# matiasrodlo/arxiv-rag

Hardware: AMD Instinct MI355X
Metric: chunks embedded/sec + QPS@top-10, all-mpnet-base-v2 768-d, 1/2/4/8 MI355X (higher is better)
Workload: dtype bf16

## Files before the change

arxiv_rag_amd/csrc/encoder_kernels.h:

```cpp
#pragma once
#include <type_traits>

#include "arx_common.h"

__global__ void scan_lens_kernel(const int32_t* __restrict__ lens, int32_t* __restrict__ cu, int n) {
    __shared__ int32_t part[1024];
    const int tid = threadIdx.x, nt = blockDim.x;
    const int per = (n + nt - 1) / nt;
    const int b0 = tid * per, b1 = min(n, b0 + per);
    int s = 0;
    for (int b = b0; b < b1; ++b) s += lens[b];
    part[tid] = s;
    __syncthreads();
    if (tid == 0) {
        int run = 0;
        for (int i = 0; i < nt; ++i) { int v = part[i]; part[i] = run; run += v; }
        cu[n] = run;
    }
    __syncthreads();
    int run = part[tid];
    for (int b = b0; b < b1; ++b) { cu[b] = run; run += lens[b]; }
}

template <int ARCH, bool SEG = false>
// ... 144 lines not shown
    constexpr int CPR = DH / 8;
    constexpr int RPB = 256 / (DH * 2);
    constexpr int KS = DH / 16;
    constexpr int DB = DH / 32;
    extern __shared__ __attribute__((aligned(16))) char smem[];

    const int b = blockIdx.z, h = blockIdx.y;
    const int t0 = cu[b];
    const int L = cu[b + 1] - t0;
    const int q0 = blockIdx.x * (32 * NW);
    if (q0 >= L) return;
    const int Lk = (L + 31) & ~31;
    const int tid = threadIdx.x, lane = tid & 63, wid = tid >> 6;
    const int64_t ld = 3 * (int64_t)H;
    const uint16_t* Qg = qkv + (int64_t)t0 * ld + h * DH;
    const uint16_t* Kg = Qg + H;
    const uint16_t* Vg = Qg + 2 * H;

    char* Ks = smem;
    uint16_t* Vt = reinterpret_cast<uint16_t*>(smem + AttnSmem<DH>::k_bytes(Lk));
    float* Bs = reinterpret_cast<float*>(smem + AttnSmem<DH>::k_bytes(Lk) + AttnSmem<DH>::vt_bytes(Lk));
    const int vts = AttnSmem<DH>::vt_stride(Lk);
    const int bst = AttnSmem<DH>::bias_stride(Lk);

    for (int cid = tid; cid < Lk * CPR; cid += NT) {
        const int row = cid / CPR, pc = cid % CPR;
        const int c = pc ^ ((row / RPB) & (CPR - 1));
        u32x4 kv = u32x4{0u, 0u, 0u, 0u}, vv = u32x4{0u, 0u, 0u, 0u};
        if (row < L) {
            kv = *reinterpret_cast<const u32x4*>(Kg + (int64_t)row * ld + c * 8);
            vv = *reinterpret_cast<const u32x4*>(Vg + (int64_t)row * ld + pc * 8);
        }
        *reinterpret_cast<u32x4*>(Ks + (int64_t)cid * 16) = kv;
        const int k16 = row & 15;
        const int pos = (row & ~15) + (((k16 >> 2) & 1) << 3) + ((k16 >> 3) << 2) + (k16 & 3);
#pragma unroll
        for (int e = 0; e < 4; ++e) {
            Vt[(pc * 8 + 2 * e) * vts + pos] = (uint16_t)(vv[e] & 0xffffu);
            Vt[(pc * 8 + 2 * e + 1) * vts + pos] = (uint16_t)(vv[e] >> 16);
        }
    }
    if (HAS_BIAS) {
        const float* bt = bias_tbl + (int64_t)h * ARX_BIAS_ROW + ARX_BIAS_CENTER;
        for (int i = tid; i < 4 * bst; i += NT) {
            const int c = i / bst, j = i % bst;
            int d = j + c - Lk;
            d = d < -ARX_BIAS_CENTER ? -ARX_BIAS_CENTER : (d > ARX_BIAS_CENTER ? ARX_BIAS_CENTER : d);
            Bs[i] = bt[d];
        }
    }
    __syncthreads();

    const int qw = q0 + wid * 32;
    if (qw >= L) return;
    const int ql = lane & 31, hh = lane >> 5;
    const int q = qw + ql;
    const int qc = q < L ? q : L - 1;
    bf16x8 qf[KS];
#pragma unroll
    for (int ks = 0; ks < KS; ++ks)
        qf[ks] = *reinterpret_cast<const bf16x8*>(Qg + (int64_t)qc * ld + ks * 16 + hh * 8);

    f32x16 o[DB];
#pragma unroll
    for (int d = 0; d < DB; ++d)
#pragma unroll
        for (int r = 0; r < 16; ++r) o[d][r] = 0.f;
    float m_run = -INFINITY, l_run = 0.f;

    const int bc = (4 - (qc & 3)) & 3;
    const float* brow = Bs + bc * bst + (Lk - qc - bc);
    const int krow_sw = ((ql / RPB) & (CPR - 1));

    const int nkt = Lk >> 5;
    for (int kt = 0; kt < nkt; ++kt) {
        f32x16 s;
#pragma unroll
        for (int r = 0; r < 16; ++r) s[r] = 0.f;
        const char* krow = Ks + (int64_t)(kt * 32 + ql) * (DH * 2);
#pragma unroll
        for (int ks = 0; ks < KS; ++ks) {
            const bf16x8 kf = *reinterpret_cast<const bf16x8*>(krow + (((2 * ks + hh) ^ krow_sw) << 4));
            s = __builtin_amdgcn_mfma_f32_32x32x16_bf16(kf, qf[ks], s, 0, 0, 0);
        }
        float mx = -INFINITY;
#pragma unroll
        for (int g4 = 0; g4 < 4; ++g4) {
            const int kb = kt * 32 + 8 * g4 + 4 * hh;
            f32x4 bv = f32x4{0.f, 0.f, 0.f, 0.f};
            if (HAS_BIAS) bv = *reinterpret_cast<const f32x4*>(brow + kb);
#pragma unroll
            for (int e = 0; e < 4; ++e) {
                float v = s[g4 * 4 + e] * scale_log2e + bv[e];
                v = (kb + e < L) ? v : -INFINITY;
                s[g4 * 4 + e] = v;
                mx = fmaxf(mx, v);
            }
        }
        mx = fmaxf(mx, __shfl_xor(mx, 32));
        const float m_new = fmaxf(m_run, mx);
        const float alpha = exp2f(m_run - m_new);
        m_run = m_new;
        float rs = 0.f;
#pragma unroll
        for (int r = 0; r < 16; ++r) { s[r] = exp2f(s[r] - m_new); rs += s[r]; }
        l_run = l_run * alpha + rs;
#pragma unroll
        for (int d = 0; d < DB; ++d)
#pragma unroll
            for (int r = 0; r < 16; ++r) o[d][r] *= alpha;
        bf16x8 pf[2];
#pragma unroll
        for (int ss = 0; ss < 2; ++ss)
#pragma unroll
            for (int e = 0; e < 8; ++e) pf[ss][e] = (bf16_t)s[8 * ss + e];
#pragma unroll
        for (int d = 0; d < DB; ++d) {
            const uint16_t* vrow = Vt + (int64_t)(d * 32 + ql) * vts + kt * 32 + hh * 8;
#pragma unroll
            for (int ss = 0; ss < 2; ++ss) {
                const bf16x8 vf = *reinterpret_cast<const bf16x8*>(vrow + ss * 16);
                o[d] = __builtin_amdgcn_mfma_f32_32x32x16_bf16(vf, pf[ss], o[d], 0, 0, 0);
            }
        }
    }
    const float l_tot = l_run + __shfl_xor(l_run, 32);
    const float inv = 1.0f / l_tot;
    if (q < L) {
        uint16_t* orow = ctx + (int64_t)(t0 + q) * H + h * DH;
#pragma unroll
        for (int d = 0; d < DB; ++d)
#pragma unroll
            for (int g4 = 0; g4 < 4; ++g4) {
                u32x2 w2;
                w2[0] = pack_bf16x2(o[d][g4 * 4 + 0] * inv, o[d][g4 * 4 + 1] * inv);
                w2[1] = pack_bf16x2(o[d][g4 * 4 + 2] * inv, o[d][g4 * 4 + 3] * inv);
                *reinterpret_cast<u32x2*>(orow + d * 32 + 8 * g4 + 4 * hh) = w2;
            }
    }
}

typedef short s16x4 __attribute__((ext_vector_type(4)));
template <int DH> struct AttnSmem2 {
    static __host__ __device__ int kv_bytes(int Lk) { return Lk * DH * 2; }
    static __host__ __device__ int bias_stride(int Lk) { return 2 * Lk + 8; }
    static __host__ __device__ int total(int Lk, bool has) { return 2 * kv_bytes(Lk) + (has ? 4 * (2 * Lk + 8) * 4 : 0); }
};

template <int DH> struct AttnSmem3 {
    static __host__ __device__ int kv_bytes(int Lk) { return Lk * DH * 2; }
    static __host__ __device__ int bias_stride(int Lk) { return ((2 * Lk + 8 + 63) & ~63) + 64; }
    static __host__ __device__ int total(int Lk, bool has) { return 2 * kv_bytes(Lk) + (has ? 4 * bias_stride(Lk) * 4 : 0); }
};
__device__ __forceinline__ int attn_bias_off(int c) { return c == 0 ? 0 : (c == 1 ? 20 : (c == 2 ? 36 : 52)); }

template <int DH, bool HAS_BIAS, int NW>
__global__ __launch_bounds__(NW * 64, NW / 2) void attention_tr_kernel(const uint16_t* __restrict__ qkv, uint16_t* __restrict__ ctx,
                                                                        const int32_t* __restrict__ cu,
                                                                        const float* __restrict__ bias_tbl, int H,
                                                                        float scale_log2e, int dev_word, unsigned long long* dev_stamps) {
    constexpr int NT = NW * 64;
    constexpr int CPR = DH / 8;
    constexpr int RPB = 256 / (DH * 2);
#ifdef ARX_DEV_VARIANTS
    const unsigned lin = blockIdx.x + gridDim.x * (blockIdx.y + gridDim.y * blockIdx.z);
    if (dev_stamps && threadIdx.x == 0) {
        dev_stamps[4 * lin] = wall_clock64();
        dev_stamps[4 * lin + 3] = ((unsigned long long)__builtin_amdgcn_s_getreg((31 << 11) | 20) << 32) | (unsigned)__builtin_amdgcn_s_getreg((31 << 11) | 4);
    }
#endif
    constexpr int KS = DH / 16;
    constexpr int DB = DH / 32;
    constexpr int ROWB = DH * 2;
    constexpr int RPI = NT / CPR;
    extern __shared__ __attribute__((aligned(16))) char smem[];
    const int b = blockIdx.z, h = blockIdx.y;
    const int t0 = cu[b];
    const int L = cu[b + 1] - t0;
    const int q0 = blockIdx.x * (32 * NW);
    if (q0 >= L) return;
    const int Lk = (L + 31) & ~31;
    const int tid = threadIdx.x, lane = tid & 63, wid = tid >> 6;
    const uint32_t ld = 3u * (uint32_t)H;
    const uint16_t* Qg = qkv + (int64_t)t0 * ld + h * DH;
    const uint16_t* Kg = Qg + H;
    const uint16_t* Vg = Qg + 2 * H;
    char* Ks = smem;
    char* Vs = smem + AttnSmem3<DH>::kv_bytes(Lk);
    float* Bs = reinterpret_cast<float*>(smem + 2 * AttnSmem3<DH>::kv_bytes(Lk));
    const int bst = AttnSmem3<DH>::bias_stride(Lk);

    const int ql = lane & 31, hh = lane >> 5;
    const int qw = q0 + wid * 32;
    const int q = qw + ql;
    const int qc = q < L ? q : L - 1;
    bf16x8 qf[KS];
#pragma unroll
    for (int ks = 0; ks < KS; ++ks)
        qf[ks] = *reinterpret_cast<const bf16x8*>(Qg + (uint32_t)qc * ld + ks * 16 + hh * 8);
    {
        static_assert(RPI % 16 == 0, "staging pass must keep the swizzle terms constant per thread");
        typedef __attribute__((address_space(3))) void lds_v;
        typedef const __attribute__((address_space(1))) void gbl_v;
        const int pc = tid % CPR, r0 = tid / CPR;
        const int kc = pc ^ ((r0 / RPB) & (CPR - 1));
        const int vc = (DH == 64) ? (pc ^ (((r0 >> 1) & 1) << 2)) : pc;
        uint32_t lo = (uint32_t)(tid & ~63) * 16;
        int LkS = Lk;
#ifdef ARX_DEV_VARIANTS
        if (dev_word == 5) LkS = 0;
#endif
        for (int row = r0; row < LkS; row += RPI, lo += NT * 16) {
            const uint32_t gr = (uint32_t)(row < L ? row : L - 1) * ld;
            __builtin_amdgcn_global_load_lds((gbl_v*)(Kg + gr + kc * 8), (lds_v*)(Ks + lo), 16, 0, 0);
            __builtin_amdgcn_global_load_lds((gbl_v*)(Vg + gr + vc * 8), (lds_v*)(Vs + lo), 16, 0, 0);
        }
    }
    if (HAS_BIAS) {
        const float* bt = bias_tbl + (int64_t)h * ARX_BIAS_ROW + ARX_BIAS_CENTER;
        const int span = 2 * Lk + 8;
        for (int i = tid; i < 4 * span; i += NT) {
            const int c = (i >= span) + (i >= 2 * span) + (i >= 3 * span), j = i - c * span;
            int d = j + c - Lk;
            d = d < -ARX_BIAS_CENTER ? -ARX_BIAS_CENTER : (d > ARX_BIAS_CENTER ? ARX_BIAS_CENTER : d);
            Bs[c * bst + attn_bias_off(c) + j] = bt[d];
        }
    }
    __syncthreads();
#ifdef ARX_DEV_VARIANTS
    if (dev_stamps && threadIdx.x == 0) dev_stamps[4 * lin + 1] = wall_clock64();
    if (dev_word == 3) {
        if (q < L && qf[0][0] == 0x7fc1 && qf[1 % KS][1] == 0x7fc2) ctx[(int64_t)(t0 + q) * H + h * DH] = 1;
        return;
    }
#endif

    if (qw >= L) return;
    f32x16 o[DB];
    auto lds_bases = [&](const float*& bb, const char* (&kb)[KS], const char* (&vb)[DB]) {
        int lane = threadIdx.x & 63;
        asm volatile("" : "+v"(lane));
        const int ql = lane & 31, hh = lane >> 5;
        int qc = q0 + wid * 32 + ql;
        qc = qc < L ? qc : L - 1;
        const int bc = (4 - (qc & 3)) & 3;
        bb = Bs + bc * bst + attn_bias_off(bc) + (Lk - qc - bc) + 4 * hh;
        const int krow_sw = ((ql / RPB) & (CPR - 1));
#pragma unroll
        for (int ks = 0; ks < KS; ++ks) kb[ks] = Ks + ql * ROWB + (((2 * ks + hh) ^ krow_sw) << 4);
        const int g16 = lane >> 4, q_ = (lane & 15) >> 2, p_ = lane & 3;
        const int vsw = (DH == 64) ? (((q_ >> 1) & 1) << 2) : 0;
#pragma unroll
        for (int d = 0; d < DB; ++d) {
            const int col = 32 * d + 16 * (g16 & 1) + 4 * p_;
            vb[d] = Vs + (4 * hh + q_) * ROWB + (((col >> 3) ^ vsw) << 4) + ((p_ & 1) << 3);
        }
    };
    typedef __attribute__((address_space(3))) s16x4 lds_s16x4;
    typedef short s16x8 __attribute__((ext_vector_type(8)));
    f32x4 lsum;
    const s16x4 one4 = s16x4{0x3f80, 0x3f80, 0x3f80, 0x3f80};
    const int nkt = Lk >> 5;
    const int nfull = (L & 31) ? nkt - 1 : nkt;
    float l_tot;

    bool redo = false;
#ifdef ARX_DEV_VARIANTS
    redo = dev_word == 6;
#endif
    if (!redo) {
#pragma unroll
        for (int d = 0; d < DB; ++d)
#pragma unroll
            for (int r = 0; r < 16; ++r) o[d][r] = 0.f;
        lsum = f32x4{0.f, 0.f, 0.f, 0.f};
        typedef const __attribute__((address_space(3))) char* lds_cptr;
        typedef const __attribute__((address_space(3))) float* lds_fptr;
        lds_fptr bp;
        lds_cptr kp[KS], vp[DB];
        {
            const float* bb;
            const char* kb[KS];
            const char* vb[DB];
            lds_bases(bb, kb, vb);
            bp = (lds_fptr)bb;
#pragma unroll
            for (int ks = 0; ks < KS; ++ks) kp[ks] = (lds_cptr)kb[ks];
#pragma unroll
            for (int d = 0; d < DB; ++d) vp[d] = (lds_cptr)vb[d];
        }
        bf16x8 kf[KS];
#pragma unroll
        for (int ks = 0; ks < KS; ++ks) kf[ks] = *reinterpret_cast<const __attribute__((address_space(3))) bf16x8*>(kp[ks]);
        auto advance = [&](int n) {
            bp += 32 * n;
            asm volatile("" : "+v"(bp));
#pragma unroll
            for (int ks = 0; ks < KS; ++ks) { kp[ks] += 32 * ROWB * n; asm volatile("" : "+v"(kp[ks])); }
#pragma unroll
            for (int d = 0; d < DB; ++d) { vp[d] += 32 * ROWB * n; asm volatile("" : "+v"(vp[d])); }
            __builtin_amdgcn_sched_barrier(0);
        };
        auto fast = [&](auto masked_tag, auto off_tag, int kt) {
            constexpr bool MASKED = decltype(masked_tag)::value;
            constexpr int OFF = decltype(off_tag)::value;
            f32x16 s;
#pragma unroll
            for (int r = 0; r < 16; ++r) s[r] = 0.f;
#pragma unroll
            for (int ks = 0; ks < KS; ++ks) s = __builtin_amdgcn_mfma_f32_32x32x16_bf16(kf[ks], qf[ks], s, 0, 0, 0);
            __builtin_amdgcn_sched_barrier(0);
            f32x4 bv[4];
#pragma unroll
            for (int g4 = 0; g4 < 4; ++g4) bv[g4] = HAS_BIAS ? *reinterpret_cast<const __attribute__((address_space(3))) f32x4*>(bp + OFF * 32 + 8 * g4) : f32x4{0.f, 0.f, 0.f, 0.f};
            s16x4 vt[DB][4];
#pragma unroll
            for (int d = 0; d < DB; ++d)
#pragma unroll
                for (int j = 0; j < 4; ++j) vt[d][j] = __builtin_amdgcn_ds_read_tr16_b64_v4i16((lds_s16x4*)(vp[d] + (OFF * 32 + 8 * j) * ROWB));
            __builtin_amdgcn_sched_barrier(0);
            typedef float f32x2 __attribute__((ext_vector_type(2)));
            const f32x2 sc2 = f32x2{scale_log2e, scale_log2e};
#pragma unroll
            for (int g4 = 0; g4 < 4; ++g4)
#pragma unroll
                for (int e = 0; e < 4; e += 2) {
                    f32x2 v = __builtin_elementwise_fma(f32x2{s[g4 * 4 + e], s[g4 * 4 + e + 1]}, sc2, f32x2{bv[g4][e], bv[g4][e + 1]});
                    if (MASKED) {
                        v[0] = (kt * 32 + 8 * g4 + 4 * hh + e < L) ? v[0] : -INFINITY;
                        v[1] = (kt * 32 + 8 * g4 + 4 * hh + e + 1 < L) ? v[1] : -INFINITY;
                    }
                    s[g4 * 4 + e] = v[0]; s[g4 * 4 + e + 1] = v[1];
                }
            __builtin_amdgcn_sched_barrier(0);
#pragma unroll
            for (int r = 0; r < 16; ++r) s[r] = __builtin_amdgcn_exp2f(s[r]);
            uint32_t pw[8];
#pragma unroll
            for (int j = 0; j < 8; ++j) pw[j] = pack_bf16x2(s[2 * j], s[2 * j + 1]);
            __builtin_amdgcn_sched_barrier(0);
            if (!MASKED) {
#pragma unroll
                for (int ks = 0; ks < KS; ++ks) kf[ks] = *reinterpret_cast<const __attribute__((address_space(3))) bf16x8*>(kp[ks] + (OFF + 1) * 32 * ROWB);
            }
            __builtin_amdgcn_sched_barrier(0);
            bf16x8 pf[2];
#pragma unroll
            for (int ss = 0; ss < 2; ++ss) pf[ss] = __builtin_bit_cast(bf16x8, u32x4{pw[4 * ss], pw[4 * ss + 1], pw[4 * ss + 2], pw[4 * ss + 3]});
#pragma unroll
            for (int j = 0; j < 4; ++j)
                lsum = __builtin_amdgcn_mfma_f32_4x4x4bf16_1k(one4, __builtin_bit_cast(s16x4, u32x2{pw[2 * j], pw[2 * j + 1]}), lsum, 0, 0, 0);
#pragma unroll
            for (int d = 0; d < DB; ++d)
#pragma unroll
                for (int ss = 0; ss < 2; ++ss) {
                    s16x8 v8;
#pragma unroll
                    for (int e = 0; e < 4; ++e) { v8[e] = vt[d][2 * ss][e]; v8[4 + e] = vt[d][2 * ss + 1][e]; }
                    o[d] = __builtin_amdgcn_mfma_f32_32x32x16_bf16(__builtin_bit_cast(bf16x8, v8), pf[ss], o[d], 0, 0, 0);
                }
            __builtin_amdgcn_sched_barrier(0);
        };
        int kt = 0;
        for (; kt + 2 <= nfull; kt += 2) {
            fast(std::false_type{}, std::integral_constant<int, 0>{}, kt);
            fast(std::false_type{}, std::integral_constant<int, 1>{}, kt + 1);
            advance(2);
        }
        if (kt < nfull) { fast(std::false_type{}, std::integral_constant<int, 0>{}, kt); advance(1); }
        if (nfull < nkt) fast(std::true_type{}, std::integral_constant<int, 0>{}, nkt - 1);
        l_tot = lsum[0] + __shfl_xor(lsum[0], 32);
        redo = !__all(l_tot > 0x1p-100f && l_tot < 0x1p100f);
    }
    if (redo) {
#pragma unroll
    for (int d = 0; d < DB; ++d)
#pragma unroll
        for (int r = 0; r < 16; ++r) o[d][r] = 0.f;
    float m_run = -INFINITY;
    const float* bptr;
    const char* kptr[KS];
    const char* vptr[DB];
    lds_bases(bptr, kptr, vptr);
    constexpr float THR = 8.0f;
    const float inv_scale = 1.0f / scale_log2e;
    lsum = f32x4{0.f, 0.f, 0.f, 0.f};
    auto tile = [&](auto masked_tag, auto first_tag, int kt) {
        constexpr bool MASKED = decltype(masked_tag)::value;
        constexpr bool FIRST = decltype(first_tag)::value;
        f32x16 s;
        const float s0 = FIRST ? 0.f : -m_run * inv_scale;
#pragma unroll
        for (int r = 0; r < 16; ++r) s[r] = s0;
#pragma unroll
        for (int ks = 0; ks < KS; ++ks) {
            const bf16x8 kf = *reinterpret_cast<const bf16x8*>(kptr[ks]);
            s = __builtin_amdgcn_mfma_f32_32x32x16_bf16(kf, qf[ks], s, 0, 0, 0);
        }
#pragma unroll
        for (int g4 = 0; g4 < 4; ++g4) {
            f32x4 bv = f32x4{0.f, 0.f, 0.f, 0.f};
            if (HAS_BIAS) bv = *reinterpret_cast<const f32x4*>(bptr + 8 * g4);
#pragma unroll
            for (int e = 0; e < 4; ++e) {
                float v = fmaf(s[g4 * 4 + e], scale_log2e, bv[e]);
                if (MASKED) v = (kt * 32 + 8 * g4 + 4 * hh + e < L) ? v : -INFINITY;
                s[g4 * 4 + e] = v;
            }
        }
        float mx = -INFINITY;
#pragma unroll
        for (int r = 0; r < 16; r += 2) mx = fmaxf(mx, fmaxf(s[r], s[r + 1]));
        mx = fmaxf(mx, __shfl_xor(mx, 32));
        if (FIRST) {
            m_run = mx;
#pragma unroll
            for (int r = 0; r < 16; ++r) s[r] -= mx;
        } else if (__any(mx > THR)) {
            const float d = fmaxf(mx, 0.f);
            const float alpha = __builtin_amdgcn_exp2f(-d);
            m_run += d;
#pragma unroll
            for (int r = 0; r < 16; ++r) s[r] -= d;
#pragma unroll
            for (int r = 0; r < 4; ++r) lsum[r] *= alpha;
#pragma unroll
            for (int dd = 0; dd < DB; ++dd)
#pragma unroll
                for (int r = 0; r < 16; ++r) o[dd][r] *= alpha;
        }
#pragma unroll
        for (int r = 0; r < 16; ++r) s[r] = __builtin_amdgcn_exp2f(s[r]);
        uint32_t pw[8];
#pragma unroll
        for (int j = 0; j < 8; ++j) pw[j] = pack_bf16x2(s[2 * j], s[2 * j + 1]);
        bf16x8 pf[2];
#pragma unroll
        for (int ss = 0; ss < 2; ++ss) pf[ss] = __builtin_bit_cast(bf16x8, u32x4{pw[4 * ss], pw[4 * ss + 1], pw[4 * ss + 2], pw[4 * ss + 3]});
#pragma unroll
        for (int j = 0; j < 4; ++j)
            lsum = __builtin_amdgcn_mfma_f32_4x4x4bf16_1k(one4, __builtin_bit_cast(s16x4, u32x2{pw[2 * j], pw[2 * j + 1]}), lsum, 0, 0, 0);
#pragma unroll
        for (int d = 0; d < DB; ++d) {
#pragma unroll
            for (int ss = 0; ss < 2; ++ss) {
                const s16x4 lo = __builtin_amdgcn_ds_read_tr16_b64_v4i16((lds_s16x4*)(vptr[d] + (16 * ss) * ROWB));
                const s16x4 hi = __builtin_amdgcn_ds_read_tr16_b64_v4i16((lds_s16x4*)(vptr[d] + (16 * ss + 8) * ROWB));
                s16x8 v8;
#pragma unroll
                for (int e = 0; e < 4; ++e) { v8[e] = lo[e]; v8[4 + e] = hi[e]; }
                o[d] = __builtin_amdgcn_mfma_f32_32x32x16_bf16(__builtin_bit_cast(bf16x8, v8), pf[ss], o[d], 0, 0, 0);
            }
        }
        bptr += 32;
#pragma unroll
        for (int ks = 0; ks < KS; ++ks) kptr[ks] += 32 * ROWB;
#pragma unroll
        for (int d = 0; d < DB; ++d) vptr[d] += 32 * ROWB;
    };
    if (nfull > 0) tile(std::false_type{}, std::true_type{}, 0); else tile(std::true_type{}, std::true_type{}, 0);
    for (int kt = 1; kt < nfull; ++kt) tile(std::false_type{}, std::false_type{}, kt);
    if (nfull < nkt && nkt > 1) tile(std::true_type{}, std::false_type{}, nkt - 1);
    l_tot = lsum[0] + __shfl_xor(lsum[0], 32);
    }

    const float inv = 1.0f / l_tot;
    u32x4 pc[DB][2];
#pragma unroll
    for (int d = 0; d < DB; ++d) {
        uint32_t w[4][2];
#pragma unroll
        for (int g4 = 0; g4 < 4; ++g4) {
            w[g4][0] = pack_bf16x2(o[d][g4 * 4 + 0] * inv, o[d][g4 * 4 + 1] * inv);
            w[g4][1] = pack_bf16x2(o[d][g4 * 4 + 2] * inv, o[d][g4 * 4 + 3] * inv);
        }
#pragma unroll
        for (int g = 0; g < 2; ++g)
#pragma unroll
            for (int k = 0; k < 2; ++k) {
                const auto sw = __builtin_amdgcn_permlane32_swap(w[g][k], w[g + 2][k], false, false);
                pc[d][g][k] = sw[0]; pc[d][g][2 + k] = sw[1];
            }
    }
    if (q < L) {
        uint16_t* orow = ctx + (int64_t)(t0 + q) * H + h * DH + 16 * hh;
#pragma unroll
        for (int d = 0; d < DB; ++d) {
            *reinterpret_cast<u32x4*>(orow + d * 32) = pc[d][0];
            *reinterpret_cast<u32x4*>(orow + d * 32 + 8) = pc[d][1];
        }
    }
#ifdef ARX_DEV_VARIANTS
    if (dev_stamps && (threadIdx.x & 63) == 0) atomicMax(&dev_stamps[4 * lin + 2], (unsigned long long)wall_clock64());
#endif
}

#ifdef ARX_DEV_VARIANTS
template <int DH, int NSLOT_ = 8> struct AttnRing {
    static constexpr int NT = 512, NSLOT = NSLOT_, AHEAD = NSLOT - 1, SLOT_KEYS = 64;
    static constexpr int ROWB = DH * 2;
    static constexpr int SLOT_BYTES = 2 * SLOT_KEYS * ROWB;
    static constexpr int GPS = SLOT_BYTES / (NT * 16);
    static_assert(GPS >= 1 && GPS * NT * 16 == SLOT_BYTES, "slot must be whole passes of the block");
    static __host__ __device__ int bias_stride(int C0) { return (2 * C0 + 8 + 52 + 63) & ~63; }
    static __host__ __device__ int total(int C0, bool has) { return NSLOT * SLOT_BYTES + (has ? 4 * bias_stride(C0) * 4 : 0); }
};

#define ARX_VMCNT_CASE(N) case N: asm volatile("s_waitcnt vmcnt(" #N ")" ::: "memory"); break;
#define ARX_VMCNT_CASE4(A, B, C_, D) ARX_VMCNT_CASE(A) ARX_VMCNT_CASE(B) ARX_VMCNT_CASE(C_) ARX_VMCNT_CASE(D)
__device__ __forceinline__ void attn_wait_vm(int n) {
    switch (n) {
    ARX_VMCNT_CASE4(0, 1, 2, 3) ARX_VMCNT_CASE4(4, 5, 6, 7) ARX_VMCNT_CASE4(8, 9, 10, 11) ARX_VMCNT_CASE4(12, 13, 14, 15)
    ARX_VMCNT_CASE4(16, 17, 18, 19) ARX_VMCNT_CASE4(20, 21, 22, 23) ARX_VMCNT_CASE4(24, 25, 26, 27) ARX_VMCNT_CASE4(28, 29, 30, 31)
    ARX_VMCNT_CASE4(32, 33, 34, 35) ARX_VMCNT_CASE4(36, 37, 38, 39) ARX_VMCNT_CASE4(40, 41, 42, 43) ARX_VMCNT_CASE(44)
    default: asm volatile("s_waitcnt vmcnt(0)" ::: "memory"); break;
    }
}
#undef ARX_VMCNT_CASE4
#undef ARX_VMCNT_CASE

template <int DH, int NSLOT> struct AttnStream {
    using R = AttnRing<DH, NSLOT>;
    static constexpr int NT = R::NT, ROWB = R::ROWB, SLOT_BYTES = R::SLOT_BYTES, GPS = R::GPS, CPR = DH / 8, RPB = 256 / R::ROWB;
    const uint16_t* qkv; const int32_t* cu; char* ring;
    int H, h, G, n_seqs;
    uint32_t ld;
    int p_b, p_t0, p_L, p_step, p_nqp, p_nsteps, p_slot, c_slot;
    int inflight, pend_st;
    unsigned st_bits;

    __device__ __forceinline__ void p_load_item() {
        p_L = 0; p_step = 0;
        while (p_b < n_seqs) {
            const __attribute__((address_space(4))) int32_t* cuc = (const __attribute__((address_space(4))) int32_t*)cu;
            const int t0 = cuc[p_b], L = cuc[p_b + 1] - t0;
            if (L > 0) { p_t0 = t0; p_L = L; p_nqp = L > 128 ? 2 : 1; p_nsteps = p_nqp + ((L + 63) >> 6); break; }
            p_b += G;
        }
    }
    __device__ __forceinline__ void issue_next() {
        const uint16_t* base = qkv + (int64_t)p_t0 * ld + h * DH;
        const bool isq = p_step < p_nqp;
        const int r0 = isq ? 128 * p_step : 64 * (p_step - p_nqp);
        int t = threadIdx.x;
        asm volatile("" : "+v"(t));
        char* dst = ring + p_slot * SLOT_BYTES + (__builtin_amdgcn_readfirstlane(t) & ~63) * 16;
#pragma unroll
        for (int it = 0; it < GPS; ++it) {
            const int cid = it * NT + t, r128 = cid / CPR, pcn = cid % CPR;
            int row, col0, c;
            if (isq) { row = r0 + r128; col0 = 0; c = pcn ^ ((r128 / RPB) & (CPR - 1)); }
            else if (r128 < 64) { row = r0 + r128; col0 = H; c = pcn ^ ((r128 / RPB) & (CPR - 1)); }
            else { row = r0 + r128 - 64; col0 = 2 * H; c = (DH == 64) ? (pcn ^ (((r128 >> 1) & 1) << 2)) : pcn; }
            row = row < p_L ? row : p_L - 1;
            __builtin_amdgcn_global_load_lds((const __attribute__((address_space(1))) void*)(base + (uint32_t)row * ld + col0 + c * 8),
                                             (__attribute__((address_space(3))) void*)(dst + it * NT * 16), 16, 0, 0);
        }
        if (pend_st) st_bits |= 1u << inflight;
        pend_st = 0;
        ++inflight;
        p_slot = (p_slot + 1) & (R::NSLOT - 1);
        if (++p_step == p_nsteps) { p_b += G; p_load_item(); }
    }
    __device__ __forceinline__ const char* step_begin() {
        attn_wait_vm((inflight - 1) * GPS + (DH / 8) * __builtin_popcount(st_bits >> 1) + pend_st);
        asm volatile("" ::: "memory");
        __builtin_amdgcn_s_barrier();
        asm volatile("" ::: "memory");
        st_bits >>= 1;
        --inflight;
        if (p_L > 0) issue_next();
        const char* slot = ring + c_slot * SLOT_BYTES;
        c_slot = (c_slot + 1) & (R::NSLOT - 1);
        return slot;
    }
};

template <int DH, bool HAS_BIAS, bool MASKED, bool first>
__device__ __forceinline__ void attn_ring_tile(const char* kbase, int k0, int v0, const bf16x8 (&qf)[DH / 16], f32x16 (&o)[DH / 32],
                                               f32x4& lsum, float& m_run, const float* bp, int kt, int hh, int L,
                                               float scale_log2e, float inv_scale) {
    constexpr int KS = DH / 16, DB = DH / 32, ROWB = DH * 2;
    constexpr float THR = 8.0f;
    typedef __attribute__((address_space(3))) s16x4 lds_s16x4;
    typedef short s16x8 __attribute__((ext_vector_type(8)));
    f32x16 s;
    const float s0 = first ? 0.f : -m_run * inv_scale;
#pragma unroll
    for (int r = 0; r < 16; ++r) s[r] = s0;
#pragma unroll
    for (int ks = 0; ks < KS; ++ks) {
        const bf16x8 kf = *reinterpret_cast<const bf16x8*>(kbase + (k0 ^ (ks << 5)));
        s = __builtin_amdgcn_mfma_f32_32x32x16_bf16(kf, qf[ks], s, 0, 0, 0);
    }
#pragma unroll
    for (int g4 = 0; g4 < 4; ++g4) {
        f32x4 bv = f32x4{0.f, 0.f, 0.f, 0.f};
        if (HAS_BIAS) bv = *reinterpret_cast<const f32x4*>(bp + 8 * g4);
#pragma unroll
        for (int e = 0; e < 4; ++e) {
            float v = fmaf(s[g4 * 4 + e], scale_log2e, bv[e]);
            if (MASKED) v = (kt * 32 + 8 * g4 + 4 * hh + e < L) ? v : -INFINITY;
            s[g4 * 4 + e] = v;
        }
    }
    float mx = -INFINITY;
#pragma unroll
    for (int r = 0; r < 16; r += 2) mx = fmaxf(mx, fmaxf(s[r], s[r + 1]));
    mx = fmaxf(mx, __shfl_xor(mx, 32));
    if (first) {
        m_run = mx;
#pragma unroll
        for (int r = 0; r < 16; ++r) s[r] -= mx;
    } else if (__any(mx > THR)) {
        const float d = fmaxf(mx, 0.f);
        const float alpha = __builtin_amdgcn_exp2f(-d);
        m_run += d;
#pragma unroll
        for (int r = 0; r < 16; ++r) s[r] -= d;
#pragma unroll
        for (int r = 0; r < 4; ++r) lsum[r] *= alpha;
#pragma unroll
        for (int dd = 0; dd < DB; ++dd)
#pragma unroll
            for (int r = 0; r < 16; ++r) o[dd][r] *= alpha;
    }
#pragma unroll
    for (int r = 0; r < 16; ++r) s[r] = __builtin_amdgcn_exp2f(s[r]);
    uint32_t pw[8];
#pragma unroll
    for (int j = 0; j < 8; ++j) pw[j] = pack_bf16x2(s[2 * j], s[2 * j + 1]);
    bf16x8 pf[2];
#pragma unroll
    for (int ss = 0; ss < 2; ++ss) pf[ss] = __builtin_bit_cast(bf16x8, u32x4{pw[4 * ss], pw[4 * ss + 1], pw[4 * ss + 2], pw[4 * ss + 3]});
    const s16x4 one4 = s16x4{0x3f80, 0x3f80, 0x3f80, 0x3f80};
#pragma unroll
    for (int j = 0; j < 4; ++j)
        lsum = __builtin_amdgcn_mfma_f32_4x4x4bf16_1k(one4, __builtin_bit_cast(s16x4, u32x2{pw[2 * j], pw[2 * j + 1]}), lsum, 0, 0, 0);
    const uint32_t vaddr = (uint32_t)(size_t)(const __attribute__((address_space(3))) char*)kbase + (uint32_t)v0;
#pragma unroll
    for (int d = 0; d < DB; ++d) {
        const uint32_t va = vaddr ^ (uint32_t)(d << 6);
        s16x4 vt[2][2];
#pragma unroll
        for (int ss = 0; ss < 2; ++ss) {
            asm volatile("ds_read_b64_tr_b16 %0, %1 offset:%2" : "=v"(vt[ss][0]) : "v"(va), "n"((16 * ss) * ROWB));
            asm volatile("ds_read_b64_tr_b16 %0, %1 offset:%2" : "=v"(vt[ss][1]) : "v"(va), "n"((16 * ss + 8) * ROWB));
        }
        asm volatile("s_waitcnt lgkmcnt(0)" : "+v"(vt[0][0]), "+v"(vt[0][1]), "+v"(vt[1][0]), "+v"(vt[1][1]) :: "memory");
#pragma unroll
        for (int ss = 0; ss < 2; ++ss) {
            s16x8 v8;
#pragma unroll
            for (int e = 0; e < 4; ++e) { v8[e] = vt[ss][0][e]; v8[4 + e] = vt[ss][1][e]; }
            o[d] = __builtin_amdgcn_mfma_f32_32x32x16_bf16(__builtin_bit_cast(bf16x8, v8), pf[ss], o[d], 0, 0, 0);
        }
    }
}

template <int DH, bool HAS_BIAS, int NSLOT>
__global__ __launch_bounds__(512, 2) void attention_ring_kernel(const uint16_t* __restrict__ qkv, uint16_t* __restrict__ ctx,
                                                                 const int32_t* __restrict__ cu,
                                                                 const float* __restrict__ bias_tbl, int H, int n_seqs,
                                                                 int C0, float scale_log2e) {
    using R = AttnRing<DH, NSLOT>;
    constexpr int NT = R::NT, ROWB = R::ROWB, SLOT_BYTES = R::SLOT_BYTES, GPS = R::GPS;
    constexpr int CPR = DH / 8;
    constexpr int RPB = 256 / ROWB;
    constexpr int KS = DH / 16;
    constexpr int DB = DH / 32;
    constexpr int NSTORE = DB * 4;
    static_assert((R::AHEAD - 1) * GPS + 4 * NSTORE <= 44, "attn_wait_vm covers AHEAD - 1 younger slot-loads plus four items' stores");
// ... 576 lines not shown
```

Measured before the change: 22410.

## Split attention K/V staging so first QK tile overlaps the V load

The attention prologue now issues all K loads before all V loads and fetches Q and bias values into registers with inline asm. It then waits only on the K portion (vmcnt of the V count) before the first barrier, so the first tile's QK^T, softmax and packing run while V is still in flight. A second barrier waits for V before the PV step, and the main loop is restructured into phase-tagged halves. The gain is overlap of global-to-LDS staging with compute, at the cost of an extra block barrier, hand-managed waitcnts, and assumptions about sequence length bounds (NB sized for 544 keys).

```diff
diff --git a/arxiv_rag_amd/csrc/encoder_kernels.h b/arxiv_rag_amd/csrc/encoder_kernels.h
--- a/arxiv_rag_amd/csrc/encoder_kernels.h
+++ b/arxiv_rag_amd/csrc/encoder_kernels.h
@@ -320,7 +320,20 @@
     static __host__ __device__ int bias_stride(int Lk) { return ((2 * Lk + 8 + 63) & ~63) + 64; }
     static __host__ __device__ int total(int Lk, bool has) { return 2 * kv_bytes(Lk) + (has ? 4 * bias_stride(Lk) * 4 : 0); }
 };
-__device__ __forceinline__ int attn_bias_off(int c) { return c == 0 ? 0 : (c == 1 ? 20 : (c == 2 ? 36 : 52)); }
+__device__ __forceinline__ int attn_bias_off(int c) { return c == 0 ? 0 : 16 * c + 4; }
+
+#define ARX_VMCNT_CASE(N) case N: asm volatile("s_waitcnt vmcnt(" #N ")" ::: "memory"); break;
+#define ARX_VMCNT_CASE4(A, B, C_, D) ARX_VMCNT_CASE(A) ARX_VMCNT_CASE(B) ARX_VMCNT_CASE(C_) ARX_VMCNT_CASE(D)
+__device__ __forceinline__ void attn_wait_vm(int n) {
+    switch (n) {
+    ARX_VMCNT_CASE4(0, 1, 2, 3) ARX_VMCNT_CASE4(4, 5, 6, 7) ARX_VMCNT_CASE4(8, 9, 10, 11) ARX_VMCNT_CASE4(12, 13, 14, 15)
+    ARX_VMCNT_CASE4(16, 17, 18, 19) ARX_VMCNT_CASE4(20, 21, 22, 23) ARX_VMCNT_CASE4(24, 25, 26, 27) ARX_VMCNT_CASE4(28, 29, 30, 31)
+    ARX_VMCNT_CASE4(32, 33, 34, 35) ARX_VMCNT_CASE4(36, 37, 38, 39) ARX_VMCNT_CASE4(40, 41, 42, 43) ARX_VMCNT_CASE(44)
+    default: asm volatile("s_waitcnt vmcnt(0)" ::: "memory"); break;
+    }
+}
+#undef ARX_VMCNT_CASE4
+#undef ARX_VMCNT_CASE
 
 template <int DH, bool HAS_BIAS, int NW>
 __global__ __launch_bounds__(NW * 64, NW / 2) void attention_tr_kernel(const uint16_t* __restrict__ qkv, uint16_t* __restrict__ ctx,
@@ -333,14 +346,15 @@
 #ifdef ARX_DEV_VARIANTS
     const unsigned lin = blockIdx.x + gridDim.x * (blockIdx.y + gridDim.y * blockIdx.z);
     if (dev_stamps && threadIdx.x == 0) {
-        dev_stamps[4 * lin] = wall_clock64();
-        dev_stamps[4 * lin + 3] = ((unsigned long long)__builtin_amdgcn_s_getreg((31 << 11) | 20) << 32) | (unsigned)__builtin_amdgcn_s_getreg((31 << 11) | 4);
+        dev_stamps[5 * lin] = wall_clock64();
+        dev_stamps[5 * lin + 3] = ((unsigned long long)__builtin_amdgcn_s_getreg((31 << 11) | 20) << 32) | (unsigned)__builtin_amdgcn_s_getreg((31 << 11) | 4);
     }
 #endif
     constexpr int KS = DH / 16;
     constexpr int DB = DH / 32;
     constexpr int ROWB = DH * 2;
     constexpr int RPI = NT / CPR;
+    constexpr int NB = (4 * (2 * 544 + 8) + NT - 1) / NT;
     extern __shared__ __attribute__((aligned(16))) char smem[];
     const int b = blockIdx.z, h = blockIdx.y;
     const int t0 = cu[b];
@@ -357,54 +371,8 @@
     char* Vs = smem + AttnSmem3<DH>::kv_bytes(Lk);
     float* Bs = reinterpret_cast<float*>(smem + 2 * AttnSmem3<DH>::kv_bytes(Lk));
     const int bst = AttnSmem3<DH>::bias_stride(Lk);
-
-    const int ql = lane & 31, hh = lane >> 5;
-    const int qw = q0 + wid * 32;
-    const int q = qw + ql;
-    const int qc = q < L ? q : L - 1;
-    bf16x8 qf[KS];
-#pragma unroll
-    for (int ks = 0; ks < KS; ++ks)
-        qf[ks] = *reinterpret_cast<const bf16x8*>(Qg + (uint32_t)qc * ld + ks * 16 + hh * 8);
-    {
-        static_assert(RPI % 16 == 0, "staging pass must keep the swizzle terms constant per thread");
-        typedef __attribute__((address_space(3))) void lds_v;
-        typedef const __attribute__((address_space(1))) void gbl_v;
-        const int pc = tid % CPR, r0 = tid / CPR;
-        const int kc = pc ^ ((r0 / RPB) & (CPR - 1));
-        const int vc = (DH == 64) ? (pc ^ (((r0 >> 1) & 1) << 2)) : pc;
-        uint32_t lo = (uint32_t)(tid & ~63) * 16;
-        int LkS = Lk;
-#ifdef ARX_DEV_VARIANTS
-        if (dev_word == 5) LkS = 0;
-#endif
-        for (int row = r0; row < LkS; row += RPI, lo += NT * 16) {
-            const uint32_t gr = (uint32_t)(row < L ? row : L - 1) * ld;
-            __builtin_amdgcn_global_load_lds((gbl_v*)(Kg + gr + kc * 8), (lds_v*)(Ks + lo), 16, 0, 0);
-            __builtin_amdgcn_global_load_lds((gbl_v*)(Vg + gr + vc * 8), (lds_v*)(Vs + lo), 16, 0, 0);
-        }
-    }
-    if (HAS_BIAS) {
-        const float* bt = bias_tbl + (int64_t)h * ARX_BIAS_ROW + ARX_BIAS_CENTER;
-        const int span = 2 * Lk + 8;
-        for (int i = tid; i < 4 * span; i += NT) {
-            const int c = (i >= span) + (i >= 2 * span) + (i >= 3 * span), j = i - c * span;
-            int d = j + c - Lk;
-            d = d < -ARX_BIAS_CENTER ? -ARX_BIAS_CENTER : (d > ARX_BIAS_CENTER ? ARX_BIAS_CENTER : d);
-            Bs[c * bst + attn_bias_off(c) + j] = bt[d];
-        }
-    }
-    __syncthreads();
-#ifdef ARX_DEV_VARIANTS
-    if (dev_stamps && threadIdx.x == 0) dev_stamps[4 * lin + 1] = wall_clock64();
-    if (dev_word == 3) {
-        if (q < L && qf[0][0] == 0x7fc1 && qf[1 % KS][1] == 0x7fc2) ctx[(int64_t)(t0 + q) * H + h * DH] = 1;
-        return;
-    }
-#endif
-
-    if (qw >= L) return;
-    f32x16 o[DB];
+    const int span4 = 4 * (2 * Lk + 8);
+
     auto lds_bases = [&](const float*& bb, const char* (&kb)[KS], const char* (&vb)[DB]) {
         int lane = threadIdx.x & 63;
         asm volatile("" : "+v"(lane));
@@ -424,6 +392,111 @@
             vb[d] = Vs + (4 * hh + q_) * ROWB + (((col >> 3) ^ vsw) << 4) + ((p_ & 1) << 3);
         }
     };
+    typedef const __attribute__((address_space(3))) char* lds_cptr;
+    typedef const __attribute__((address_space(3))) float* lds_fptr;
+    lds_fptr bp;
+    lds_cptr kp[KS], vp[DB];
+
+    const int ql = lane & 31, hh = lane >> 5;
+    const int qw = q0 + wid * 32;
+    const int q = qw + ql;
+    const int qc = q < L ? q : L - 1;
+    bf16x8 qf[KS];
+    {
+        u32x4 qraw[KS];
+#pragma unroll
+        for (int ks = 0; ks < KS; ++ks)
+            asm volatile("global_load_dwordx4 %0, %1, off" : "=v"(qraw[ks]) : "v"(Qg + (uint32_t)qc * ld + ks * 16 + hh * 8) : "memory");
+        float bvv[NB];
+        auto bias_slot = [&](int i, int& j) {
+            const int span = 2 * Lk + 8;
+            const int c = (i >= span) + (i >= 2 * span) + (i >= 3 * span);
+            j = i - c * span;
+            return c;
+        };
+        if (HAS_BIAS) {
+            const float* bt = bias_tbl + (int64_t)h * ARX_BIAS_ROW + ARX_BIAS_CENTER;
+#pragma unroll
+            for (int it = 0; it < NB; ++it)
+                if (it * NT < span4) {
+                    int i = tid + it * NT, j;
+                    i = i < span4 ? i : span4 - 1;
+                    const int c = bias_slot(i, j);
+                    int d = j + c - Lk;
+                    d = d < -ARX_BIAS_CENTER ? -ARX_BIAS_CENTER : (d > ARX_BIAS_CENTER ? ARX_BIAS_CENTER : d);
+                    asm volatile("global_load_dword %0, %1, off" : "=v"(bvv[it]) : "v"(bt + d) : "memory");
+                }
+        }
+        static_assert(RPI % 16 == 0, "staging pass must keep the swizzle terms constant per thread");
+        static_assert(32 % (64 / CPR) == 0, "a wave's rows of one pass must not straddle a 32-row group");
+        typedef __attribute__((address_space(3))) void lds_v;
+        typedef const __attribute__((address_space(1))) void gbl_v;
+        const int pc = tid % CPR, r0 = tid / CPR;
+        const int kc = pc ^ ((r0 / RPB) & (CPR - 1));
+        const int vc = (DH == 64) ? (pc ^ (((r0 >> 1) & 1) << 2)) : pc;
+        const uint32_t lo = (uint32_t)(tid & ~63) * 16;
+        int LkS = Lk;
+#ifdef ARX_DEV_VARIANTS
+        if (dev_word == 5) LkS = 0;
+#endif
+        const int r0w = __builtin_amdgcn_readfirstlane(r0);
+        const int npc = r0w < LkS ? (LkS - r0w + RPI - 1) / RPI : 0;
+#pragma unroll 1
+        for (int p = 0; p < npc; ++p) {
+            const int row = r0 + p * RPI;
+            const uint32_t gr = (uint32_t)(row < L ? row : L - 1) * ld;
+            __builtin_amdgcn_global_load_lds((gbl_v*)(Kg + gr + kc * 8), (lds_v*)(Ks + lo + p * (NT * 16)), 16, 0, 0);
+        }
+#pragma unroll 1
+        for (int p = 0; p < npc; ++p) {
+            const int row = r0 + p * RPI;
+            const uint32_t gr = (uint32_t)(row < L ? row : L - 1) * ld;
+            __builtin_amdgcn_global_load_lds((gbl_v*)(Vg + gr + vc * 8), (lds_v*)(Vs + lo + p * (NT * 16)), 16, 0, 0);
+        }
+        uint32_t bdst[NB];
+        if (HAS_BIAS) {
+#pragma unroll
+            for (int it = 0; it < NB; ++it)
+                if (it * NT < span4) {
+                    const int i = tid + it * NT;
+                    int j;
+                    const int c = bias_slot(i < span4 ? i : span4 - 1, j);
+                    bdst[it] = (uint32_t)(size_t)(__attribute__((address_space(3))) float*)(Bs + c * bst + attn_bias_off(c) + j);
+                }
+        }
+        {
+            const float* bb;
+            const char* kb[KS];
+            const char* vb[DB];
+            lds_bases(bb, kb, vb);
+            bp = (lds_fptr)bb;
+#pragma unroll
+            for (int ks = 0; ks < KS; ++ks) kp[ks] = (lds_cptr)kb[ks];
+#pragma unroll
+            for (int d = 0; d < DB; ++d) vp[d] = (lds_cptr)vb[d];
+        }
+        __builtin_amdgcn_sched_barrier(0);
+        attn_wait_vm(npc);
+#pragma unroll
+        for (int ks = 0; ks < KS; ++ks) {
+            asm volatile("" : "+v"(qraw[ks]));
+            qf[ks] = __builtin_bit_cast(bf16x8, qraw[ks]);
+        }
+        if (HAS_BIAS) {
+#pragma unroll
+            for (int it = 0; it < NB; ++it)
+                if (it * NT < span4 && tid + it * NT < span4) asm volatile("ds_write_b32 %0, %1" :: "v"(bdst[it]), "v"(bvv[it]) : "memory");
+        }
+        asm volatile("s_waitcnt lgkmcnt(0)" ::: "memory");
+        __builtin_amdgcn_s_barrier();
+        asm volatile("" ::: "memory");
+    }
+#ifdef ARX_DEV_VARIANTS
+    if (dev_stamps && threadIdx.x == 0) dev_stamps[5 * lin + 1] = wall_clock64();
+#endif
+
+    const bool wave_on = qw < L;
+    f32x16 o[DB];
     typedef __attribute__((address_space(3))) s16x4 lds_s16x4;
     typedef short s16x8 __attribute__((ext_vector_type(8)));
     f32x4 lsum;
@@ -436,30 +509,19 @@
 #ifdef ARX_DEV_VARIANTS
     redo = dev_word == 6;
 #endif
+    auto second_barrier = [&]() {
+        __builtin_amdgcn_sched_barrier(0);
+        asm volatile("s_waitcnt vmcnt(0)" ::: "memory");
+        __builtin_amdgcn_s_barrier();
+        asm volatile("" ::: "memory");
+#ifdef ARX_DEV_VARIANTS
+        if (dev_stamps && threadIdx.x == 0) dev_stamps[5 * lin + 4] = wall_clock64();
+#endif
+    };
     if (!redo) {
-#pragma unroll
-        for (int d = 0; d < DB; ++d)
-#pragma unroll
-            for (int r = 0; r < 16; ++r) o[d][r] = 0.f;
         lsum = f32x4{0.f, 0.f, 0.f, 0.f};
-        typedef const __attribute__((address_space(3))) char* lds_cptr;
-        typedef const __attribute__((address_space(3))) float* lds_fptr;
-        lds_fptr bp;
-        lds_cptr kp[KS], vp[DB];
-        {
-            const float* bb;
-            const char* kb[KS];
-            const char* vb[DB];
-            lds_bases(bb, kb, vb);
-            bp = (lds_fptr)bb;
-#pragma unroll
-            for (int ks = 0; ks < KS; ++ks) kp[ks] = (lds_cptr)kb[ks];
-#pragma unroll
-            for (int d = 0; d < DB; ++d) vp[d] = (lds_cptr)vb[d];
-        }
         bf16x8 kf[KS];
-#pragma unroll
-        for (int ks = 0; ks < KS; ++ks) kf[ks] = *reinterpret_cast<const __attribute__((address_space(3))) bf16x8*>(kp[ks]);
+        uint32_t pw0[8];
         auto advance = [&](int n) {
             bp += 32 * n;
             asm volatile("" : "+v"(bp));
@@ -469,76 +531,118 @@
             for (int d = 0; d < DB; ++d) { vp[d] += 32 * ROWB * n; asm volatile("" : "+v"(vp[d])); }
             __builtin_amdgcn_sched_barrier(0);
         };
-        auto fast = [&](auto masked_tag, auto off_tag, int kt) {
+        auto fast = [&](auto masked_tag, auto off_tag, auto phase_tag, int kt) {
             constexpr bool MASKED = decltype(masked_tag)::value;
             constexpr int OFF = decltype(off_tag)::value;
-            f32x16 s;
-#pragma unroll
-            for (int r = 0; r < 16; ++r) s[r] = 0.f;
-#pragma unroll
-            for (int ks = 0; ks < KS; ++ks) s = __builtin_amdgcn_mfma_f32_32x32x16_bf16(kf[ks], qf[ks], s, 0, 0, 0);
-            __builtin_amdgcn_sched_barrier(0);
-            f32x4 bv[4];
-#pragma unroll
-            for (int g4 = 0; g4 < 4; ++g4) bv[g4] = HAS_BIAS ? *reinterpret_cast<const __attribute__((address_space(3))) f32x4*>(bp + OFF * 32 + 8 * g4) : f32x4{0.f, 0.f, 0.f, 0.f};
+            constexpr int PHASE = decltype(phase_tag)::value;
+            uint32_t pwt[8];
+            uint32_t (&pw)[8] = *(PHASE == 0 ? &pwt : &pw0);
             s16x4 vt[DB][4];
-#pragma unroll
-            for (int d = 0; d < DB; ++d)
-#pragma unroll
-                for (int j = 0; j < 4; ++j) vt[d][j] = __builtin_amdgcn_ds_read_tr16_b64_v4i16((lds_s16x4*)(vp[d] + (OFF * 32 + 8 * j) * ROWB));
-            __builtin_amdgcn_sched_barrier(0);
-            typedef float f32x2 __attribute__((ext_vector_type(2)));
-            const f32x2 sc2 = f32x2{scale_log2e, scale_log2e};
-#pragma unroll
-            for (int g4 = 0; g4 < 4; ++g4)
-#pragma unroll
-                for (int e = 0; e < 4; e += 2) {
-                    f32x2 v = __builtin_elementwise_fma(f32x2{s[g4 * 4 + e], s[g4 * 4 + e + 1]}, sc2, f32x2{bv[g4][e], bv[g4][e + 1]});
-                    if (MASKED) {
-                        v[0] = (kt * 32 + 8 * g4 + 4 * hh + e < L) ? v[0] : -INFINITY;
-                        v[1] = (kt * 32 + 8 * g4 + 4 * hh + e + 1 < L) ? v[1] : -INFINITY;
+            auto read_vt = [&]() {
+#pragma unroll
+                for (int d = 0; d < DB; ++d)
+#pragma unroll
+                    for (int j = 0; j < 4; ++j) vt[d][j] = __builtin_amdgcn_ds_read_tr16_b64_v4i16((lds_s16x4*)(vp[d] + (OFF * 32 + 8 * j) * ROWB));
+            };
+            if (PHASE != 2) {
+                f32x16 s;
+#pragma unroll
+                for (int r = 0; r < 16; ++r) s[r] = 0.f;
+#pragma unroll
+                for (int ks = 0; ks < KS; ++ks) s = __builtin_amdgcn_mfma_f32_32x32x16_bf16(kf[ks], qf[ks], s, 0, 0, 0);
+                __builtin_amdgcn_sched_barrier(0);
+                f32x4 bv[4];
+#pragma unroll
+                for (int g4 = 0; g4 < 4; ++g4) bv[g4] = HAS_BIAS ? *reinterpret_cast<const __attribute__((address_space(3))) f32x4*>(bp + OFF * 32 + 8 * g4) : f32x4{0.f, 0.f, 0.f, 0.f};
+                if (PHASE == 0) read_vt();
+                __builtin_amdgcn_sched_barrier(0);
+                typedef float f32x2 __attribute__((ext_vector_type(2)));
+                const f32x2 sc2 = f32x2{scale_log2e, scale_log2e};
+#pragma unroll
+                for (int g4 = 0; g4 < 4; ++g4)
+#pragma unroll
+                    for (int e = 0; e < 4; e += 2) {
+                        f32x2 v = __builtin_elementwise_fma(f32x2{s[g4 * 4 + e], s[g4 * 4 + e + 1]}, sc2, f32x2{bv[g4][e], bv[g4][e + 1]});
+                        if (MASKED) {
+                            v[0] = (kt * 32 + 8 * g4 + 4 * hh + e < L) ? v[0] : -INFINITY;
+                            v[1] = (kt * 32 + 8 * g4 + 4 * hh + e + 1 < L) ? v[1] : -INFINITY;
+                        }
+                        s[g4 * 4 + e] = v[0]; s[g4 * 4 + e + 1] = v[1];
                     }
-                    s[g4 * 4 + e] = v[0]; s[g4 * 4 + e + 1] = v[1];
+                __builtin_amdgcn_sched_barrier(0);
+#pragma unroll
+                for (int r = 0; r < 16; ++r) s[r] = __builtin_amdgcn_exp2f(s[r]);
+#pragma unroll
+                for (int j = 0; j < 8; ++j) pw[j] = pack_bf16x2(s[2 * j], s[2 * j + 1]);
+                __builtin_amdgcn_sched_barrier(0);
+                if (!MASKED) {
+#pragma unroll
+                    for (int ks = 0; ks < KS; ++ks) kf[ks] = *reinterpret_cast<const __attribute__((address_space(3))) bf16x8*>(kp[ks] + (OFF + 1) * 32 * ROWB);
                 }
-            __builtin_amdgcn_sched_barrier(0);
-#pragma unroll
-            for (int r = 0; r < 16; ++r) s[r] = __builtin_amdgcn_exp2f(s[r]);
-            uint32_t pw[8];
-#pragma unroll
-            for (int j = 0; j < 8; ++j) pw[j] = pack_bf16x2(s[2 * j], s[2 * j + 1]);
-            __builtin_amdgcn_sched_barrier(0);
-            if (!MASKED) {
-#pragma unroll
-                for (int ks = 0; ks < KS; ++ks) kf[ks] = *reinterpret_cast<const __attribute__((address_space(3))) bf16x8*>(kp[ks] + (OFF + 1) * 32 * ROWB);
-            }
-            __builtin_amdgcn_sched_barrier(0);
-            bf16x8 pf[2];
-#pragma unroll
-            for (int ss = 0; ss < 2; ++ss) pf[ss] = __builtin_bit_cast(bf16x8, u32x4{pw[4 * ss], pw[4 * ss + 1], pw[4 * ss + 2], pw[4 * ss + 3]});
-#pragma unroll
-            for (int j = 0; j < 4; ++j)
-                lsum = __builtin_amdgcn_mfma_f32_4x4x4bf16_1k(one4, __builtin_bit_cast(s16x4, u32x2{pw[2 * j], pw[2 * j + 1]}), lsum, 0, 0, 0);
-#pragma unroll
-            for (int d = 0; d < DB; ++d)
-#pragma unroll
-                for (int ss = 0; ss < 2; ++ss) {
-                    s16x8 v8;
-#pragma unroll
-                    for (int e = 0; e < 4; ++e) { v8[e] = vt[d][2 * ss][e]; v8[4 + e] = vt[d][2 * ss + 1][e]; }
-                    o[d] = __builtin_amdgcn_mfma_f32_32x32x16_bf16(__builtin_bit_cast(bf16x8, v8), pf[ss], o[d], 0, 0, 0);
+                __builtin_amdgcn_sched_barrier(0);
+            }
+            if (PHASE != 1) {
+                if (PHASE == 2) {
+                    read_vt();
+                    __builtin_amdgcn_sched_barrier(0);
                 }
-            __builtin_amdgcn_sched_barrier(0);
+                bf16x8 pf[2];
+#pragma unroll
+                for (int ss = 0; ss < 2; ++ss) pf[ss] = __builtin_bit_cast(bf16x8, u32x4{pw[4 * ss], pw[4 * ss + 1], pw[4 * ss + 2], pw[4 * ss + 3]});
+#pragma unroll
+                for (int j = 0; j < 4; ++j)
+                    lsum = __builtin_amdgcn_mfma_f32_4x4x4bf16_1k(one4, __builtin_bit_cast(s16x4, u32x2{pw[2 * j], pw[2 * j + 1]}), lsum, 0, 0, 0);
+#pragma unroll
+                for (int d = 0; d < DB; ++d)
+#pragma unroll
+                    for (int ss = 0; ss < 2; ++ss) {
+                        s16x8 v8;
+#pragma unroll
+                        for (int e = 0; e < 4; ++e) { v8[e] = vt[d][2 * ss][e]; v8[4 + e] = vt[d][2 * ss + 1][e]; }
+                        o[d] = __builtin_amdgcn_mfma_f32_32x32x16_bf16(__builtin_bit_cast(bf16x8, v8), pf[ss], o[d], 0, 0, 0);
+                    }
+                __builtin_amdgcn_sched_barrier(0);
+            }
         };
-        int kt = 0;
-        for (; kt + 2 <= nfull; kt += 2) {
-            fast(std::false_type{}, std::integral_constant<int, 0>{}, kt);
-            fast(std::false_type{}, std::integral_constant<int, 1>{}, kt + 1);
-            advance(2);
-        }
-        if (kt < nfull) { fast(std::false_type{}, std::integral_constant<int, 0>{}, kt); advance(1); }
-        if (nfull < nkt) fast(std::true_type{}, std::integral_constant<int, 0>{}, nkt - 1);
+        constexpr std::integral_constant<int, 0> T0{};
+        constexpr std::integral_constant<int, 1> T1{};
+        constexpr std::integral_constant<int, 2> PV{};
+        if (wave_on) {
+#pragma unroll
+            for (int ks = 0; ks < KS; ++ks) kf[ks] = *reinterpret_cast<const __attribute__((address_space(3))) bf16x8*>(kp[ks]);
+            if (nfull > 0) fast(std::false_type{}, T0, T1, 0); else fast(std::true_type{}, T0, T1, 0);
+#pragma unroll
+            for (int j = 0; j < 8; ++j) asm volatile("" : "+v"(pw0[j]));
+        }
+        second_barrier();
+        if (!wave_on) return;
+#ifdef ARX_DEV_VARIANTS
+        if (dev_word == 3) {
+            if (q < L && pw0[0] == 0x7fc17fc2u && pw0[7] == 0x7fc27fc1u) ctx[(int64_t)(t0 + q) * H + h * DH] = 1;
+            return;
+        }
+#endif
+#pragma unroll
+        for (int d = 0; d < DB; ++d)
+#pragma unroll
+            for (int r = 0; r < 16; ++r) o[d][r] = 0.f;
+        fast(std::false_type{}, T0, PV, 0);
+        if (nfull > 0) {
+            advance(1);
+            int kt = 1;
+            for (; kt + 2 <= nfull; kt += 2) {
+                fast(std::false_type{}, T0, T0, kt);
+                fast(std::false_type{}, T1, T0, kt + 1);
+                advance(2);
+            }
+            if (kt < nfull) { fast(std::false_type{}, T0, T0, kt); advance(1); }
+            if (nfull < nkt) fast(std::true_type{}, T0, T0, nkt - 1);
+        }
         l_tot = lsum[0] + __shfl_xor(lsum[0], 32);
         redo = !__all(l_tot > 0x1p-100f && l_tot < 0x1p100f);
+    } else {
+        second_barrier();
+        if (!wave_on) return;
     }
     if (redo) {
 #pragma unroll
@@ -659,7 +763,7 @@
         }
     }
 #ifdef ARX_DEV_VARIANTS
-    if (dev_stamps && (threadIdx.x & 63) == 0) atomicMax(&dev_stamps[4 * lin + 2], (unsigned long long)wall_clock64());
+    if (dev_stamps && (threadIdx.x & 63) == 0) atomicMax(&dev_stamps[5 * lin + 2], (unsigned long long)wall_clock64());
 #endif
 }
 
@@ -673,19 +777,6 @@
     static __host__ __device__ int bias_stride(int C0) { return (2 * C0 + 8 + 52 + 63) & ~63; }
     static __host__ __device__ int total(int C0, bool has) { return NSLOT * SLOT_BYTES + (has ? 4 * bias_stride(C0) * 4 : 0); }
 };
-
-#define ARX_VMCNT_CASE(N) case N: asm volatile("s_waitcnt vmcnt(" #N ")" ::: "memory"); break;
-#define ARX_VMCNT_CASE4(A, B, C_, D) ARX_VMCNT_CASE(A) ARX_VMCNT_CASE(B) ARX_VMCNT_CASE(C_) ARX_VMCNT_CASE(D)
-__device__ __forceinline__ void attn_wait_vm(int n) {
-    switch (n) {
-    ARX_VMCNT_CASE4(0, 1, 2, 3) ARX_VMCNT_CASE4(4, 5, 6, 7) ARX_VMCNT_CASE4(8, 9, 10, 11) ARX_VMCNT_CASE4(12, 13, 14, 15)
-    ARX_VMCNT_CASE4(16, 17, 18, 19) ARX_VMCNT_CASE4(20, 21, 22, 23) ARX_VMCNT_CASE4(24, 25, 26, 27) ARX_VMCNT_CASE4(28, 29, 30, 31)
-    ARX_VMCNT_CASE4(32, 33, 34, 35) ARX_VMCNT_CASE4(36, 37, 38, 39) ARX_VMCNT_CASE4(40, 41, 42, 43) ARX_VMCNT_CASE(44)
-    default: asm volatile("s_waitcnt vmcnt(0)" ::: "memory"); break;
-    }
-}
-#undef ARX_VMCNT_CASE4
-#undef ARX_VMCNT_CASE
 
 template <int DH, int NSLOT> struct AttnStream {
     using R = AttnRing<DH, NSLOT>;
```

After: 22320. Within noise of the previous version (-0.4%).
